# JINXER000/GIE-mapping

Measured on AMD Instinct MI355X. Metric: edt_map_update_throughput, higher is better.
Workload: dtype int32; 1 GPU; 512x512x512 @ 0.05 m, sensor-less hash world (BASELINE config 5): occupied iff hash(x,y,z) < 1 %, full observation, 25 ~; preset=c5, fast_mode=False, tiles=single volume, blocks=360448

## Files before the change

gie-mapping_amd/csrc/gie_api.inc.h:

```cpp
#include <stdio.h>
#include <stdlib.h>
#include <string.h>
#include <math.h>
#include <string>
#include <vector>

enum { GIE_K_CLASSIFY = 0, GIE_K_RAY_REGISTER, GIE_K_RAY_FREE, GIE_K_RAY_FINAL, GIE_K_ALLOC, GIE_K_FUSE, GIE_K_EDT_Y, GIE_K_EDT_X,
       GIE_K_EDT_Z, GIE_K_MARK, GIE_K_FRONTIER, GIE_K_WAVE_A, GIE_K_WAVE_B, GIE_K_WAVE_C, GIE_K_COMMIT, GIE_K_EDT_ZFACES, GIE_K_MARKC, GIE_K_NUM };
#include <cstdio>
#include <unistd.h>
static const char *const gie_kernel_names[GIE_K_NUM] = { "ogm_classify", "ray_register", "ray_free", "ray_finalize", "block_alloc", "fuse",
       "edt_pass_y", "edt_pass_x", "edt_pass_z", "mark", "frontiers", "wave_a", "wave_b", "waves", "commit", "edt_prep", "mark_commit" };

#define GIE_REHASH_PERIOD 64
static thread_local std::string g_gie_err;
static void gie_set_err(const std::string &s) { g_gie_err = s; }
extern "C" const char *gie_last_error(void) { return g_gie_err.c_str(); }

enum gie_owed {
    GIE_OWED_NONE,
    GIE_OWED_FRESH,
    GIE_OWED_STALE
};
struct gie_pivots { int pvt[3], upvt[3], tb0[3]; };
// ... 762 lines not shown
}

extern "C" int gie_step(gie_mapper *m)
{
    int rc = gie_fuse(m); if (rc) return rc;
    rc = gie_batch_edt(m); if (rc) return rc;
    return gie_merge(m);
}

static int gie_fetch_counters(gie_mapper *m)
{
    be_d2h(&m->be, m->h_cnt, m->c.cnt, sizeof(m->h_cnt));
    const int e = m->h_cnt[GIE_CNT_ERR];
    {
        static const int dbg = GIE_SWITCH("GIE_DEBUG_COUNTS", 0);
        if (dbg) fprintf(stderr, "gie counts: tiles known %d, frontier tiles %d, fuse tiles %d, seeds A/B/C %d %d %d, tiles without a read of the stored records %d, tiles caught up %d, lazy tiles written out %d\n", m->h_cnt[GIE_CNT_TL_KNOWN],
                         m->h_cnt[GIE_CNT_TL_FRONT], m->h_cnt[GIE_CNT_TL_FUSE], m->h_cnt[GIE_CNT_SEED_A], m->h_cnt[GIE_CNT_SEED_B], m->h_cnt[GIE_CNT_SEED_C], m->h_cnt[GIE_CNT_TSKIP],
                         m->h_cnt[GIE_CNT_STATE1], m->h_cnt[GIE_CNT_STATE2]);
    }
    if (e & ~GIE_ERRF_BARRIER) {
        std::string s = "device capacity exceeded:";
        if (e & GIE_ERRF_POOL) s += " block pool (raise gie_config.max_blocks)";
        if (e & GIE_ERRF_QUEUE) s += " frontier queue";
        if (e & GIE_ERRF_HASH) s += " hash table";
        gie_set_err(s);
        return GIE_ERR_CAPACITY;
    }
    if (e & GIE_ERRF_BARRIER) {
        be_memset(&m->be, &m->c.cnt[GIE_CNT_ERR], 0, sizeof(int32_t));
        be_sync(&m->be);
        gie_set_err("grid barrier of the wavefront kernel timed out (its workgroups were not all resident: another process is holding the "
                    "device); this map update is incomplete, the next one runs normally");
        return GIE_ERR_TIMEOUT;
// ... 488 lines not shown
```

gie-mapping_amd/csrc/gie_hip.hip:

```cpp
#include <cstdio>
#include <unistd.h>
#include <cstring>
#include <cstdlib>
#include <string>
#include <algorithm>
#include <vector>
#include <hip/hip_runtime.h>
#include <hip/hip_ext.h>
#include <rocprim/rocprim.hpp>
#include "gie_kernels.hip.h"

#define GIE_NEV 8

struct be_state {
    int device;
    int num_cu;
    int cu_total;
    hipStream_t stream;
    hipEvent_t ev[GIE_NEV];
    int ev_set[GIE_NEV];
    void *scan_tmp; size_t scan_bytes;
    void *arena;
    hipEvent_t copy_ev[2];
    hipStream_t side;
// ... 282 lines not shown
{
    constexpr int LP = 64 * CP;
    const size_t tile = ((size_t)c.Z * (TX + 1) + 3) & ~(size_t)3;
    const size_t lds = tile * 4 + (size_t)WAVES * LP * 8 + (size_t)LP * 2 + 16;
    static bool attr_done = false;
    if (!attr_done) {
        GIE_HIP_OK(hipFuncSetAttribute(reinterpret_cast<const void *>(&k_edt_z<CP, TX, WAVES>), hipFuncAttributeMaxDynamicSharedMemorySize, 160 * 1024));
        attr_done = true;
    }
    const int ntx = (c.X + TX - 1) / TX, ntiles = ntx * c.Y;
    int wgs = (int)((160 * 1024) / (lds + 256));
    if (wgs < 1) wgs = 1; if (wgs > 4) wgs = 4;
    int grid = wgs * b->cu_total; if (grid > (ntiles + 1) / 2) grid = (ntiles + 1) / 2;
    GIE_LAUNCH(b, (k_edt_z<CP, TX, WAVES>), dim3(grid), dim3(64 * WAVES), lds, c, ntx, ntiles, full);
}
template <int CP> static void gie_launch_edt_xz(be_state *b, const gie_ctx &c, bool zpass, int full)
{
    if (!zpass) {
        GIE_LAUNCH(b, k_edt_x<CP>, dim3((c.Y + GIE_EDTX_WAVES - 1) / GIE_EDTX_WAVES, c.Z), dim3(64 * GIE_EDTX_WAVES), 0, c);
    } else {
        gie_launch_edt_z<CP, 16, 8>(b, c, full);
    }
}
static void gie_launch_edt_dim(be_state *b, const gie_ctx &c, int L, bool zpass, int full)
{
    if (L <= 64) gie_launch_edt_xz<1>(b, c, zpass, full);
    else if (L <= 128) gie_launch_edt_xz<2>(b, c, zpass, full);
    else if (L <= 256) gie_launch_edt_xz<4>(b, c, zpass, full);
    else if (L <= 512) gie_launch_edt_xz<8>(b, c, zpass, full);
    else gie_launch_edt_xz<16>(b, c, zpass, full);
}
static int be_edt_z_stream(be_state *b, const gie_ctx &c, int full);
static void be_edt_z(be_state *b, const gie_ctx &c, int full) { (void)be_edt_z_stream(b, c, full); gie_launch_edt_dim(b, c, c.Z, true, full); }
template <bool STAGED, class F> static void be_vox_list(be_state *b, const gie_ctx &c, const F &f, const int32_t *list, int count_idx, int always_list, int lx = 64)
{
    static const int mult = GIE_SWITCH("GIE_VOXA_MULT", 32);
    const dim3 g(b->cu_total * mult), t(256);
    if (lx == 32) GIE_LAUNCH(b, (k_voxa<F, STAGED, 32>), g, t, 0, c, f, list, count_idx, always_list);
    else if (lx == 16) GIE_LAUNCH(b, (k_voxa<F, STAGED, 16>), g, t, 0, c, f, list, count_idx, always_list);
    else if (lx == 8) GIE_LAUNCH(b, (k_voxa<F, STAGED, 8>), g, t, 0, c, f, list, count_idx, always_list);
    else GIE_LAUNCH(b, (k_voxa<F, STAGED, 64>), g, t, 0, c, f, list, count_idx, always_list);
}
static void be_markc(be_state *b, const gie_ctx &c, const int32_t *list)
{
    static const int generic = GIE_SWITCH("GIE_MARKC_GENERIC", 0);
    static const int lx = GIE_SWITCH("GIE_MARKC_LX", 32);
    static const int mult = GIE_SWITCH("GIE_VOXA_MULT", 64);
    if (generic) { be_vox_list<true>(b, c, op_markc(), list, GIE_CNT_TL_KNOWN, 0, lx == 16 || lx == 8 || lx == 32 ? lx : 64); return; }
// ... 47 lines not shown
    GIE_LAUNCH(b, k_frontier_faces, dim3(nsum + nface), dim3(64 * GIE_FF_WAVES), 0, c, fp, known, known_idx, nsum);
    static int mult = GIE_SWITCH("GIE_FRONT_MULT", 0);
    if (mult <= 0) {
        int per_cu = 0;
        if (hipOccupancyMaxActiveBlocksPerMultiprocessor(&per_cu, reinterpret_cast<const void *>(&k_frontier_tiles), 64 * GIE_FR_WAVES, 0) != hipSuccess || per_cu < 1) per_cu = 2;
        mult = per_cu;
    }
    GIE_LAUNCH(b, k_frontier_tiles, dim3(b->cu_total * mult), dim3(64 * GIE_FR_WAVES), 0, c, list, count_idx);
}
static void be_edt_z_direct(be_state *b, const gie_ctx &c)
{
    GIE_LAUNCH(b, k_edt_z_direct, dim3(b->cu_total * 16), dim3(256), 0, c);
}
static int be_edt_z_stream(be_state *b, const gie_ctx &c, int full)
{
    if (c.Z < 64 || c.Z > 1024) return 0;
    static const int on = GIE_SWITCH("GIE_ZSTREAM", 1);
    if (!on) return 0;
    const int nxr = (c.X + 63) / 64;
    static const int target = GIE_SWITCH("GIE_ZSTREAM_WAVES", 8);
    const long long want = (long long)b->cu_total * 4 * target;
    int nseg = (int)((want + (long long)nxr * c.Y - 1) / ((long long)nxr * c.Y));
    const int maxseg = c.Z / 64 > 0 ? c.Z / 64 : 1;
    if (nseg > maxseg) nseg = maxseg; if (nseg < 1) nseg = 1;
    int seg_len = ((c.Z + nseg - 1) / nseg + 31) & ~31;
    nseg = (c.Z + seg_len - 1) / seg_len;
    const long long waves = (long long)nxr * nseg * c.Y;
    long long grid = (waves + 3) / 4;
    const long long cap = (long long)b->cu_total * 8 * 4;
    if (grid > cap) grid = cap;
    if (!full && grid < (long long)b->cu_total * 16) grid = (long long)b->cu_total * 16;
    GIE_LAUNCH(b, k_edt_z_stream, dim3((unsigned)grid), dim3(256), 0, c, full, nseg, seg_len);
    return 1;
}
static void be_tile_oldskip(be_state *b, const gie_ctx &c, const int pupvt[3])
{
    const int ntile = c.tfd[0] * c.tfd[1] * c.tfd[2];
    int32_t *const count = &c.cnt[GIE_CNT_STATE1];
    GIE_LAUNCH(b, k_tile_oldskip, dim3((ntile + 255) / 256), dim3(256), 0, c, ntile, c.wc_list[0], count);
    if (c.catchup_fast) GIE_LAUNCH(b, k_coc_catchup_new, dim3(b->cu_total * 8), dim3(256), 0, c, pupvt[0], pupvt[1], pupvt[2], c.wc_list[0], count);
}
static void be_pair_materialise(be_state *b, const gie_ctx &c, int stay)
{
    const int ntile = c.tfd[0] * c.tfd[1] * c.tfd[2];
    int32_t *const count = &c.cnt[GIE_CNT_STATE2];
    GIE_LAUNCH(b, k_pair_lazy_list, dim3((ntile + 255) / 256), dim3(256), 0, c, ntile, stay, c.wc_list[1], count);
    GIE_LAUNCH(b, k_pair_lazy_run, dim3(b->cu_total * 8), dim3(256), 0, c, c.wc_list[1], count);
// ... 17 lines not shown
    be_prof(b, 6, 0);
    static const int y4 = GIE_SWITCH("GIE_EDTY4", 1);
    if (y4 && (c.X & 3) == 0) {
        const int yb = c.Y > 512 ? 32 : 16, nq = (c.Y + yb - 1) / yb;
        const int lanes = (y4 == 3) ? 32 : 16;
        dim3 g4((c.X / 4 + lanes - 1) / lanes, c.Z), b4(lanes, nq);
        if (yb == 16 && lanes == 16) GIE_LAUNCH(b, (k_edt_y4<16, 16>), g4, b4, 0, c);
        else if (yb == 16) GIE_LAUNCH(b, (k_edt_y4<16, 32>), g4, b4, 0, c);
        else if (lanes == 16) GIE_LAUNCH(b, (k_edt_y4<32, 16>), g4, b4, 0, c);
        else GIE_LAUNCH(b, (k_edt_y4<32, 32>), g4, b4, 0, c);
    }
    else if (c.Y <= 256) GIE_LAUNCH(b, (k_edt_y<8, 8>), gy, dim3(GIE_EDTY_COLS, 8), 0, c);
    else if (c.Y <= 512) GIE_LAUNCH(b, (k_edt_y<16, 16>), gy, dim3(GIE_EDTY_COLS, 16), 0, c);
    else GIE_LAUNCH(b, (k_edt_y<32, 16>), gy, dim3(GIE_EDTY_COLS, 16), 0, c);
    be_prof(b, 6, 1);
    be_prof(b, 7, 0); gie_launch_edt_dim(b, c, c.X, false, 1); be_prof(b, 7, 1);
    be_prof(b, 8, 0);
    if (!be_edt_z_stream(b, c, full) && !full) be_edt_z_direct(b, c);
    gie_launch_edt_dim(b, c, c.Z, true, full);
    be_prof(b, 8, 1);

}
static void be_waves(be_state *b, const gie_ctx &c, int with_ab, int record_seeds, int clear_first)
{
    std::lock_guard<std::mutex> lock(g_waves_mutex);
    const int dv = b->device & 63;
    (void)hipSetDevice(b->device);
    const bool chain = g_live_mappers[dv] > 1;
    if (chain) {
        if (g_waves_event_set[dv]) GIE_HIP_OK(hipStreamWaitEvent(b->stream, g_waves_event[dv], 0));
        else { GIE_HIP_OK(hipEventCreateWithFlags(&g_waves_event[dv], hipEventDisableTiming)); g_waves_event_set[dv] = true; }
    }
    if (clear_first) {
        GIE_HIP_OK(hipMemsetAsync(&c.cnt[GIE_CNT_BAR_B], 0, 2 * sizeof(int32_t), b->stream));
// ... 9 lines not shown
```

gie-mapping_amd/csrc/gie_kernels.hip.h:

```cpp
#ifndef GIE_KERNELS_HIP_H
#define GIE_KERNELS_HIP_H

#include <hip/hip_runtime.h>
#include "gie_functors.h"

#if defined(GIE_WAVE_TIMING) || defined(GIE_RAY_TIMING)
#include "../../tools/measure/gie_timing.h"
#endif
#if !defined(GIE_WAVE_TIMING)
#define GIE_TS2(tag, n) do { } while (0)
#define GIE_WPROF_DECL do { } while (0)
#define GIE_WPROF_MARK(base) do { } while (0)
#define GIE_WPROF_ADD(i, v) do { } while (0)
#define GIE_WPROF_END(base) do { } while (0)
#define GIE_WPROF_DRAIN() do { } while (0)
#define GIE_WPROF_SUB(i) do { } while (0)
#define GIE_WPROF_SUBSTART() do { } while (0)
#define GIE_WPROF_DUMP() do { } while (0)
#define GIE_WPROF_CLK() 0ull
#define GIE_WAVE_TIMING_RESET(cond) do { } while (0)
#endif
#if !defined(GIE_RAY_TIMING)
#define GIE_RTS(k) do { } while (0)
#endif
// ... 689 lines not shown

__device__ __forceinline__ int gie_row_compact_push(uint2 *ce, int base, const bool valid, const uint32_t a, const int i, const uint32_t hi16, const int lane, int2 *mb = nullptr)
{
    const unsigned long long m = __ballot(valid);
    if (valid) {
        const int j = base + __popcll(m & ((1ull << lane) - 1ull));
        ce[j] = make_uint2((a << 10) | (uint32_t)j, ((uint32_t)i << 5) | (hi16 << 16));
        if (mb && j < GIE_BAND_MAXK) mb[j] = make_int2(-(i << 11), (int)((((uint32_t)(i * i) + a) << 10) | (uint32_t)j));
    }
    return base + __popcll(m);
}

#ifndef GIE_EDTX_WAVES
#define GIE_EDTX_WAVES 4
#endif
template <int CP>
__global__ __launch_bounds__(64 * GIE_EDTX_WAVES) void k_edt_x(const gie_ctx c)
{
    constexpr int LP = 64 * CP;
    __shared__ __attribute__((aligned(16))) uint2 s_ce[GIE_EDTX_WAVES][LP];
    constexpr bool OVL = LP >= 2 * (GIE_BAND_MAXK + GIE_BAND_PAD) && LP / 2 >= GIE_BAND_MAXK;
    __shared__ __attribute__((aligned(16))) int2 s_mb[OVL ? 1 : GIE_EDTX_WAVES][OVL ? 1 : GIE_BAND_MAXK + GIE_BAND_PAD];
    const int wave = threadIdx.x >> 6, lane = threadIdx.x & 63;
    const int z = blockIdx.y, y = blockIdx.x * GIE_EDTX_WAVES + wave;
    if (!c.zocc[z]) return;
    if (y >= c.Y) return;
    const int X = c.X;
    const size_t row = (size_t)z * c.Y + y;
    const uint16_t *in = c.cy1 + row * X;
    uint2 *ce = s_ce[wave];
    int2 *mb = OVL ? reinterpret_cast<int2 *>(ce + LP / 2) : s_mb[OVL ? 0 : wave];
    int K = 0;
    uint16_t cyv[CP];
#pragma unroll
    for (int m = 0; m < CP; m++) { const int i = 64 * m + lane; cyv[m] = __builtin_nontemporal_load(&in[min(i, X - 1)]); }
    uint32_t *out = c.cxy2 + row * X;
    if (CP >= 4) {
        int kall = 0;
#pragma unroll
// ... 52 lines not shown
        int sj[CP];
        gie_row_argmin<CP>(ce, K, X, lane, sj);
#pragma unroll
        for (int m = 0; m < CP; m++) {
            const uint32_t e = ce[sj[m]].y;
            o[m] = ((e & 0xffffu) >> 5) | (e & 0xffff0000u);
        }
    }
    if (CP >= 4 && (X & 3) == 0) {
#pragma unroll
        for (int m = 0; m < CP; m += 4)
            if (u0 + m < X) *reinterpret_cast<uint4 *>(out + u0 + m) = make_uint4(o[m], o[m + 1 < CP ? m + 1 : m], o[m + 2 < CP ? m + 2 : m], o[m + 3 < CP ? m + 3 : m]);
    } else {
#pragma unroll
        for (int m = 0; m < CP; m++) if (u0 + m < X) out[u0 + m] = o[m];
    }
}

template <int CP, int TX, int WAVES>
__global__ __launch_bounds__(64 * WAVES, (CP <= 8 ? 4 : 2)) void k_edt_z(const gie_ctx c, const int ntiles_x, const int ntiles, const int full)
{
    static_assert(TX == 16 && WAVES == 8, "a workgroup tile spans two 8-voxel tile columns, one column per wave and half");
    if (full == 0 && gie_z_use_lists(c, c.cnt[GIE_CNT_TL_KNOWN])) return;
    const int repair = c.cnt[GIE_CNT_ZSTREAM];
    if (repair && c.cnt[GIE_CNT_ZFAIL] == 0) return;
    constexpr int LP = 64 * CP;
    constexpr int TS = TX + 1;
    constexpr int NT = 64 * WAVES;
    constexpr int ZSTEP = NT / TX;
    constexpr int NLD = (LP + ZSTEP - 1) / ZSTEP;
// ... 189 lines not shown
#define GIE_ZS_C 16
#endif
#define GIE_ZS_W (GIE_ZS_C + 2 * GIE_ZS_R)
#define GIE_ZS_LDAUX 2
#define GIE_ZS_STAUX 2
#define GIE_ZS_NONE 0xb0000000u
#define GIE_ZS_LIMIT ((uint32_t)((GIE_ZS_R + 1) * (GIE_ZS_R + 1)) << 24)
__device__ __forceinline__ uint32_t gie_zs_key(const uint32_t v, const bool plane_ok, const int x8, const int y8, const int j)
{
    const uint32_t ux = (uint32_t)(x8 - (int)(v & 0xffffu)), uy = (uint32_t)(y8 - (int)(v >> 16));
    const int dx = (int)ux - 8, dy = (int)uy - 8;
    const uint32_t a = (uint32_t)(__mul24(dx, dx) + __mul24(dy, dy));
    const bool ok = plane_ok && max(ux, uy) <= 16u && a < (uint32_t)((GIE_ZS_R + 1) * (GIE_ZS_R + 1));
    return ok ? ((a << 24) | ((uint32_t)j << 18) | (ux << 13) | (uy << 8)) : (GIE_ZS_NONE | ((uint32_t)j << 18));
}
__device__ __forceinline__ void gie_edt_z_direct_body(const gie_ctx &c);
#define GIE_ZS_R2 24
__device__ __noinline__ bool gie_zs_wide_trip(const uint32_t *cxy2, uint32_t *bcoc, const unsigned nbytes, const unsigned voff, const unsigned pstride,
                                              const int zc, const int z1, const int Z, const int x, const int y, const bool inx, const uint8_t *occ)
{
    const __amdgpu_buffer_rsrc_t rs_in = __builtin_amdgcn_make_buffer_rsrc(const_cast<uint32_t *>(cxy2), 0, nbytes, 0x00020000);
    const __amdgpu_buffer_rsrc_t rs_out = __builtin_amdgcn_make_buffer_rsrc(bcoc, 0, nbytes, 0x00020000);
    uint32_t best[GIE_ZS_C];
#pragma unroll
    for (int t = 0; t < GIE_ZS_C; t++) best[t] = 0xffffffffu;
    const int lo = max(zc - GIE_ZS_R2, 0), hi = min(zc + GIE_ZS_C + GIE_ZS_R2, Z);
#pragma unroll 1
    for (int i0 = lo; i0 < hi; i0 += 8) {
        uint32_t v[8];
#pragma unroll
// ... 8 lines not shown
            for (int t = 0; t < GIE_ZS_C; t++) { const int d = zc + t - i; best[t] = min(best[t], (min(a + (uint32_t)(d * d), 0x3fffffu) << 10) | (uint32_t)i); }
        }
    }
    uint32_t worst = 0;
#pragma unroll
    for (int t = 0; t < GIE_ZS_C; t++) if (zc + t < z1) worst = max(worst, best[t]);
    if (__any(inx && worst >= ((uint32_t)((GIE_ZS_R2 + 1) * (GIE_ZS_R2 + 1)) << 10))) return false;
#pragma unroll
    for (int t = 0; t < GIE_ZS_C; t++) {
        const int sp = (int)(best[t] & 1023u);
        const uint32_t v = __builtin_amdgcn_raw_buffer_load_b32(rs_in, voff, (unsigned)sp * pstride, 0);
        __builtin_amdgcn_raw_buffer_store_b32(gie_pack_bcoc((int)(v & 0xffffu), (int)(v >> 16), sp), rs_out, (zc + t < z1) ? voff : GIE_BUF_OOB, (unsigned)min(zc + t, Z - 1) * pstride, 0);
    }
    return true;
}
__global__ __launch_bounds__(256, 6) void k_edt_z_stream(const gie_ctx c, const int full, const int nseg, const int seg_len)
{
    __shared__ uint8_t s_occ[1024 + 2 * (32 + 2 * GIE_ZS_R)];
    const int Z = c.Z, X = c.X, Y = c.Y;
    if (full == 0 && gie_z_use_lists(c, c.cnt[GIE_CNT_TL_KNOWN])) { gie_edt_z_direct_body(c); return; }
    if (*c.zcount <= GIE_BAND_MAXK) return;
    if (blockIdx.x == 0 && threadIdx.x == 0) c.cnt[GIE_CNT_ZSTREAM] = 1;
    for (int i = threadIdx.x; i < Z + 2 * GIE_ZS_W; i += 256) { const int z = i - GIE_ZS_W; s_occ[i] = (z >= 0 && z < Z) ? c.zocc[z] : (uint8_t)0; }
    __syncthreads();
    const int lane = threadIdx.x & 63;
    const int nxr = (X + 63) >> 6;
    const int total = nxr * nseg * Y;
    const size_t plane = (size_t)X * Y;
    const unsigned nbytes = (unsigned)((size_t)X * Y * Z * 4u);
    const __amdgpu_buffer_rsrc_t rs_in = __builtin_amdgcn_make_buffer_rsrc(const_cast<uint32_t *>(c.cxy2), 0, nbytes, 0x00020000);
    const __amdgpu_buffer_rsrc_t rs_out = __builtin_amdgcn_make_buffer_rsrc(c.bcoc, 0, nbytes, 0x00020000);
    const unsigned pstride = (unsigned)(plane * 4u);
    for (int w = (int)blockIdx.x * 4 + (int)(threadIdx.x >> 6); w < total; w += (int)gridDim.x * 4) {
        const int xr = w % nxr, seg = (w / nxr) % nseg, y = w / (nxr * nseg);
        const int x = xr * 64 + lane;
        const int z0 = seg * seg_len, z1 = min(Z, z0 + seg_len);
        if (z0 >= Z) continue;
        const unsigned voff = x < X ? (unsigned)(y * X + x) * 4u : GIE_BUF_OOB;
        const int x8 = x + 8, y8 = y + 8;
        uint32_t wk[GIE_ZS_W];
        {
            const int zz = z0 - GIE_ZS_R + lane;
            const unsigned long long pm = __ballot(lane < 2 * GIE_ZS_R && s_occ[zz + GIE_ZS_W] != 0);
            uint32_t v[2 * GIE_ZS_R];
#pragma unroll
            for (int j = 0; j < 2 * GIE_ZS_R; j++) { const int zp = min(max(z0 - GIE_ZS_R + j, 0), Z - 1); v[j] = __builtin_amdgcn_raw_buffer_load_b32(rs_in, voff, (unsigned)zp * pstride, 0); }
#pragma unroll
            for (int j = 0; j < 2 * GIE_ZS_R; j++) wk[j] = gie_zs_key(v[j], (pm >> j) & 1ull, x8, y8, j);
        }
        bool failed = false;
        int wide = 0, wz0 = 0, wz1 = 0;
#pragma unroll 1
        for (int zc = z0; zc < z1; zc += GIE_ZS_C) {
            {
                const int zz = zc + GIE_ZS_R + lane;
                const unsigned long long pm = __ballot(lane < GIE_ZS_C && s_occ[zz + GIE_ZS_W] != 0);
                uint32_t v[GIE_ZS_C];
#pragma unroll
                for (int j = 0; j < GIE_ZS_C; j++) { const int zp = min(zc + GIE_ZS_R + j, Z - 1); v[j] = __builtin_amdgcn_raw_buffer_load_b32(rs_in, voff, (unsigned)zp * pstride, GIE_ZS_LDAUX); }
#pragma unroll
                for (int j = 0; j < GIE_ZS_C; j++) wk[2 * GIE_ZS_R + j] = gie_zs_key(v[j], (pm >> j) & 1ull, x8, y8, 2 * GIE_ZS_R + j);
            }
            uint32_t wlo = 0, whi = 0;
#pragma unroll
            for (int t = 0; t < GIE_ZS_C; t++) {
                const int p = GIE_ZS_R + t;
                uint32_t b = wk[p];
#pragma unroll
                for (int d = 1; d <= GIE_ZS_R; d++) b = min(b, min(wk[p - d], wk[p + d]) + ((uint32_t)(d * d) << 24));
// ... 12 lines not shown
                m0 = max(m0, (uint32_t)__shfl_xor((int)m0, 4)); m1 = max(m1, (uint32_t)__shfl_xor((int)m1, 4));
                if ((lane & 7) == 0 && x < X) {
                    const int t0 = gie_tile_index(c, x, y, zc);
                    __hip_atomic_fetch_max(&c.tbmax[t0], (int32_t)m0, __ATOMIC_RELAXED, __HIP_MEMORY_SCOPE_AGENT);
                    if (zc + 8 < z1) __hip_atomic_fetch_max(&c.tbmax[t0 + c.tfd[0] * c.tfd[1]], (int32_t)m1, __ATOMIC_RELAXED, __HIP_MEMORY_SCOPE_AGENT);
                }
            }
            if (__any(x < X && worst >= GIE_ZS_LIMIT)) {
                if (wide == 2) { failed = true; break; }
                if (wide == 0) wz0 = zc; else wz1 = zc;
                wide++;
            }
#pragma unroll
            for (int j = 0; j < 2 * GIE_ZS_R; j++) wk[j] = wk[GIE_ZS_C + j] - ((uint32_t)GIE_ZS_C << 18);
        }
        if (!failed && wide > 0) failed = !gie_zs_wide_trip(c.cxy2, c.bcoc, nbytes, voff, pstride, wz0, z1, Z, x, y, x < X, s_occ + GIE_ZS_W);
        if (!failed && wide > 1) failed = !gie_zs_wide_trip(c.cxy2, c.bcoc, nbytes, voff, pstride, wz1, z1, Z, x, y, x < X, s_occ + GIE_ZS_W);
        if (failed && lane < 4) {
            const int tx16 = xr * 4 + lane;
            if (tx16 * 16 < X) c.zredo[(size_t)y * ((X + 15) >> 4) + tx16] = 1u;
            if (lane == 0) atomicAdd(&c.cnt[GIE_CNT_ZFAIL], 1);
        }
    }
}

#define GIE_PREP_WAVES 16
__global__ __launch_bounds__(64 * GIE_PREP_WAVES) void k_edt_prep(const gie_ctx c, const int ncol)
{
    if (blockIdx.x == 0 && threadIdx.x < 64) {
        uint8_t f[16];
#pragma unroll
        for (int i = 0; i < 16; i++) { const int z = 64 * i + (int)threadIdx.x; f[i] = c.zocc[min(z, c.Z - 1)]; }
        int k = 0;
#pragma unroll
        for (int i = 0; i < 16; i++) {
            const int z = 64 * i + (int)threadIdx.x;
// ... 1914 lines not shown
```

gie-mapping_amd/csrc/gie_ops.h:

```cpp
#ifndef GIE_OPS_H
#define GIE_OPS_H

#include "gie_types.h"

#ifndef GIE_PLATFORM_DEFINED
#include "gie_platform.h"
#endif

GIE_DEV void gie_push64(const gie_ctx &c, uint64_t *q, int32_t *counter, int cap, uint64_t v)
{
    const int i = gie_aadd32(counter, 1);
    if (i < cap) gie_st(&q[i], v); else gie_aor32(&c.cnt[GIE_CNT_ERR], GIE_ERRF_QUEUE);
}
GIE_DEV void gie_push64a(const gie_ctx &c, uint64_t *q, gie_vaddr *qaddr, int32_t *counter, int cap, uint64_t v, gie_vaddr a)
{
    const int i = gie_aadd32(counter, 1);
    if (i < cap) { gie_st(&q[i], v); gie_st(&qaddr[i], a); } else gie_aor32(&c.cnt[GIE_CNT_ERR], GIE_ERRF_QUEUE);
}
GIE_DEV void gie_push64a_wave(const gie_ctx &c, uint64_t *q, gie_vaddr *qaddr, int32_t *counter, int cap, bool push, uint64_t v, gie_vaddr a)
{
    const unsigned long long m = __ballot(push);
    if (!m) return;
    const int lane = __lane_id(), leader = __ffsll((long long)m) - 1;
    int base = 0;
// ... 700 lines not shown
}
GIE_DEV int gie_frontier_voxel(const gie_ctx &c, int x, int y, int z)
{
    const int id = gie_lid(c, x, y, z);
    if (c.glb_type[id] == GIE_VOX_UNKNOWN) return 0;
    gie_frontier_st s;
    gie_frontier_load1(c, id, x, y, z, s);
    return gie_frontier_finish(c, id, x, y, z, s);
}

GIE_DEV int gie_batch_dist_direct(const gie_ctx &c, int x, int y, int z)
{
    const int K = *c.zcount;
    const size_t plane = (size_t)c.X * c.Y, o = (size_t)y * c.X + x;
    int best = c.max_width * c.max_width;
    for (int j = 0; j < K; j += 8) {
        int zj[8]; uint32_t v[8];
#pragma unroll
        for (int u = 0; u < 8; u++) zj[u] = c.zlist[j + u < K ? j + u : K - 1];
#pragma unroll
        for (int u = 0; u < 8; u++) v[u] = c.cxy2[(size_t)zj[u] * plane + o];
#pragma unroll
        for (int u = 0; u < 8; u++) {
            const int dx = x - (int)(v[u] & 0xffffu), dy = y - (int)(v[u] >> 16), dz = z - zj[u];
            const int d = dx * dx + dy * dy + dz * dz;
            best = d < best ? d : best;
        }
    }
    return best;
}
// ... 526 lines not shown
```

gie-mapping_amd/csrc/gie_types.h:

```cpp
#ifndef GIE_TYPES_H
#define GIE_TYPES_H

#include <stdint.h>
#include "../../include/gie.h"
#include "../../include/gie_math.h"

#define GIE_VB 8
#define GIE_VBSZ 512
typedef long long gie_vaddr;

#define GIE_PAIR_DIST_SHIFT 42
#define GIE_PAIR_NEW (1ull << 41)
#define GIE_PAIR_PAR_MASK ((1ull << 41) - 1ull)
#define GIE_PAR_NONE GIE_PAIR_PAR_MASK
#define GIE_NOPROP 0xffffffffffffffffull

GIE_HD uint64_t gie_pair_make(int dist, uint64_t par) { return ((uint64_t)(uint32_t)dist << GIE_PAIR_DIST_SHIFT) | (par & GIE_PAIR_PAR_MASK); }
GIE_HD int gie_pair_dist(uint64_t p) { return (int)(p >> GIE_PAIR_DIST_SHIFT); }
GIE_HD uint64_t gie_pair_par(uint64_t p) { return p & GIE_PAIR_PAR_MASK; }
GIE_HD uint64_t gie_pack_wr(int x, int y, int z) { return (uint64_t)(uint32_t)x | ((uint64_t)(uint32_t)y << 14) | ((uint64_t)(uint32_t)z << 28); }
GIE_HD void gie_unpack_wr(uint64_t id, int *x, int *y, int *z)
{
    *x = (int)(id & 0x3fff); *y = (int)((id >> 14) & 0x3fff); *z = (int)((id >> 28) & 0x1fff);
    if ((id & GIE_PAIR_PAR_MASK) == GIE_PAR_NONE) *z = 0x3fff;
// ... 119 lines not shown
    uint64_t *qa, *qb;
    gie_vaddr *qa_a, *qb_a;
    int32_t *qc[2];
    int qcap_ab, qcap_c;
    int32_t *cnt;
    int32_t *lvl_next, *lvl_vis;
    int32_t *wc_list[2];
    int32_t *wc_flag[2];
    const int32_t *gate;
} gie_ctx;
#define GIE_GATE_CLOSED(c) ((c).gate != nullptr && *(const volatile int32_t *)(c).gate == 0)

enum {
    GIE_CNT_A = 0, GIE_CNT_B, GIE_CNT_C,
    GIE_CNT_TL_SWEPT,
    GIE_CNT_FREE4, GIE_CNT_FREE5,
    GIE_CNT_LV0, GIE_CNT_LV1, GIE_CNT_LV2,
    GIE_CNT_ERR,
    GIE_CNT_NEWBLK,
    GIE_CNT_VIS_A, GIE_CNT_VIS_B, GIE_CNT_VIS_C,
    GIE_CNT_LVL_A, GIE_CNT_LVL_B, GIE_CNT_LVL_C,
    GIE_CNT_FRONT_B, GIE_CNT_FRONT_C,
    GIE_CNT_SEED_A, GIE_CNT_SEED_B, GIE_CNT_SEED_C,
    GIE_CNT_ZSTREAM,
    GIE_CNT_ZFAIL,
    GIE_CNT_STATE1, GIE_CNT_STATE2,
    GIE_CNT_FRAME_END = 28,
    GIE_CNT_TOT_A = 28, GIE_CNT_TOT_B = 30, GIE_CNT_TOT_C = 32,
    GIE_CNT_BAR_B = 34,
    GIE_CNT_BAR_C = 35,
    GIE_CNT_NEWLIST = 36,
// ... 107 lines not shown
```

Baseline: 90190 Mvoxels/s.

## Fuse X-pass into Z-stream EDT using cy1 LDS rows, redo failed slabs

When the streamed Z pass will run, the X pass kernel now exits early. The Z-stream kernel instead builds its keys directly from the 16-bit cy1 plane through LDS row windows, and the wide trips read cy1 the same way. This is meant to drop the separate X-pass write and read of cxy2. Rows whose slabs fail are recomputed by a new redo X kernel, and tile max bounds are raised. gie_batch_dist_direct can now read the streamed bcoc result instead of scanning all z-slices. This adds complexity and possible correctness risk around the fallback paths.

```diff
diff --git a/gie-mapping_amd/csrc/gie_api.inc.h b/gie-mapping_amd/csrc/gie_api.inc.h
--- a/gie-mapping_amd/csrc/gie_api.inc.h
+++ b/gie-mapping_amd/csrc/gie_api.inc.h
@@ -800,9 +800,9 @@
     const int e = m->h_cnt[GIE_CNT_ERR];
     {
         static const int dbg = GIE_SWITCH("GIE_DEBUG_COUNTS", 0);
-        if (dbg) fprintf(stderr, "gie counts: tiles known %d, frontier tiles %d, fuse tiles %d, seeds A/B/C %d %d %d, tiles without a read of the stored records %d, tiles caught up %d, lazy tiles written out %d\n", m->h_cnt[GIE_CNT_TL_KNOWN],
+        if (dbg) fprintf(stderr, "gie counts: tiles known %d, frontier tiles %d, fuse tiles %d, seeds A/B/C %d %d %d, tiles without a read of the stored records %d, tiles caught up %d, lazy tiles written out %d, pass Z streamed %d (wide trips %d, slabs given up %d)\n", m->h_cnt[GIE_CNT_TL_KNOWN],
                          m->h_cnt[GIE_CNT_TL_FRONT], m->h_cnt[GIE_CNT_TL_FUSE], m->h_cnt[GIE_CNT_SEED_A], m->h_cnt[GIE_CNT_SEED_B], m->h_cnt[GIE_CNT_SEED_C], m->h_cnt[GIE_CNT_TSKIP],
-                         m->h_cnt[GIE_CNT_STATE1], m->h_cnt[GIE_CNT_STATE2]);
+                         m->h_cnt[GIE_CNT_STATE1], m->h_cnt[GIE_CNT_STATE2], m->h_cnt[GIE_CNT_ZSTREAM], m->h_cnt[GIE_CNT_ZWIDE], m->h_cnt[GIE_CNT_ZFAIL]);
     }
     if (e & ~GIE_ERRF_BARRIER) {
         std::string s = "device capacity exceeded:";
diff --git a/gie-mapping_amd/csrc/gie_hip.hip b/gie-mapping_amd/csrc/gie_hip.hip
--- a/gie-mapping_amd/csrc/gie_hip.hip
+++ b/gie-mapping_amd/csrc/gie_hip.hip
@@ -320,24 +320,38 @@
     int grid = wgs * b->cu_total; if (grid > (ntiles + 1) / 2) grid = (ntiles + 1) / 2;
     GIE_LAUNCH(b, (k_edt_z<CP, TX, WAVES>), dim3(grid), dim3(64 * WAVES), lds, c, ntx, ntiles, full);
 }
-template <int CP> static void gie_launch_edt_xz(be_state *b, const gie_ctx &c, bool zpass, int full)
-{
-    if (!zpass) {
-        GIE_LAUNCH(b, k_edt_x<CP>, dim3((c.Y + GIE_EDTX_WAVES - 1) / GIE_EDTX_WAVES, c.Z), dim3(64 * GIE_EDTX_WAVES), 0, c);
+template <int CP> static void gie_launch_edt_xz(be_state *b, const gie_ctx &c, bool zpass, int full, int zs_fused = 0, bool redo = false)
+{
+    if (redo) {
+        GIE_LAUNCH(b, k_edt_x_redo<CP>, dim3(b->cu_total * 8), dim3(64 * GIE_EDTX_WAVES), 0, c);
+    } else if (!zpass) {
+        GIE_LAUNCH(b, k_edt_x<CP>, dim3((c.Y + GIE_EDTX_WAVES - 1) / GIE_EDTX_WAVES, c.Z), dim3(64 * GIE_EDTX_WAVES), 0, c, zs_fused, full);
     } else {
         gie_launch_edt_z<CP, 16, 8>(b, c, full);
     }
 }
-static void gie_launch_edt_dim(be_state *b, const gie_ctx &c, int L, bool zpass, int full)
-{
-    if (L <= 64) gie_launch_edt_xz<1>(b, c, zpass, full);
-    else if (L <= 128) gie_launch_edt_xz<2>(b, c, zpass, full);
-    else if (L <= 256) gie_launch_edt_xz<4>(b, c, zpass, full);
-    else if (L <= 512) gie_launch_edt_xz<8>(b, c, zpass, full);
-    else gie_launch_edt_xz<16>(b, c, zpass, full);
+static void gie_launch_edt_dim(be_state *b, const gie_ctx &c, int L, bool zpass, int full, int zs_fused = 0, bool redo = false)
+{
+    if (L <= 64) gie_launch_edt_xz<1>(b, c, zpass, full, zs_fused, redo);
+    else if (L <= 128) gie_launch_edt_xz<2>(b, c, zpass, full, zs_fused, redo);
+    else if (L <= 256) gie_launch_edt_xz<4>(b, c, zpass, full, zs_fused, redo);
+    else if (L <= 512) gie_launch_edt_xz<8>(b, c, zpass, full, zs_fused, redo);
+    else gie_launch_edt_xz<16>(b, c, zpass, full, zs_fused, redo);
+}
+static int be_zs_mode(const gie_ctx &c)
+{
+    if (c.Z < 64 || c.Z > 1024) return 0;
+    static const int on = GIE_SWITCH("GIE_ZSTREAM", 1);
+    static const int fused = GIE_SWITCH("GIE_ZS_FUSED", 1);
+    return on ? ((fused && (c.X & 1) == 0) ? 2 : 1) : 0;
 }
 static int be_edt_z_stream(be_state *b, const gie_ctx &c, int full);
-static void be_edt_z(be_state *b, const gie_ctx &c, int full) { (void)be_edt_z_stream(b, c, full); gie_launch_edt_dim(b, c, c.Z, true, full); }
+static void be_edt_z_rest(be_state *b, const gie_ctx &c, int full, int zs)
+{
+    if (zs == 2) gie_launch_edt_dim(b, c, c.X, false, full, 0, true);
+    gie_launch_edt_dim(b, c, c.Z, true, full);
+}
+static void be_edt_z(be_state *b, const gie_ctx &c, int full) { be_edt_z_rest(b, c, full, be_edt_z_stream(b, c, full) ? be_zs_mode(c) : 0); }
 template <bool STAGED, class F> static void be_vox_list(be_state *b, const gie_ctx &c, const F &f, const int32_t *list, int count_idx, int always_list, int lx = 64)
 {
     static const int mult = GIE_SWITCH("GIE_VOXA_MULT", 32);
@@ -415,9 +429,8 @@
 }
 static int be_edt_z_stream(be_state *b, const gie_ctx &c, int full)
 {
-    if (c.Z < 64 || c.Z > 1024) return 0;
-    static const int on = GIE_SWITCH("GIE_ZSTREAM", 1);
-    if (!on) return 0;
+    const int zs = be_zs_mode(c);
+    if (!zs) return 0;
     const int nxr = (c.X + 63) / 64;
     static const int target = GIE_SWITCH("GIE_ZSTREAM_WAVES", 8);
     const long long want = (long long)b->cu_total * 4 * target;
@@ -431,7 +444,8 @@
     const long long cap = (long long)b->cu_total * 8 * 4;
     if (grid > cap) grid = cap;
     if (!full && grid < (long long)b->cu_total * 16) grid = (long long)b->cu_total * 16;
-    GIE_LAUNCH(b, k_edt_z_stream, dim3((unsigned)grid), dim3(256), 0, c, full, nseg, seg_len);
+    if (zs == 2) GIE_LAUNCH(b, k_edt_z_stream<true>, dim3((unsigned)grid), dim3(256), 0, c, full, nseg, seg_len, zs);
+    else GIE_LAUNCH(b, k_edt_z_stream<false>, dim3((unsigned)grid), dim3(256), 0, c, full, nseg, seg_len, zs);
     return 1;
 }
 static void be_tile_oldskip(be_state *b, const gie_ctx &c, const int pupvt[3])
@@ -479,10 +493,12 @@
     else if (c.Y <= 512) GIE_LAUNCH(b, (k_edt_y<16, 16>), gy, dim3(GIE_EDTY_COLS, 16), 0, c);
     else GIE_LAUNCH(b, (k_edt_y<32, 16>), gy, dim3(GIE_EDTY_COLS, 16), 0, c);
     be_prof(b, 6, 1);
-    be_prof(b, 7, 0); gie_launch_edt_dim(b, c, c.X, false, 1); be_prof(b, 7, 1);
+    const int zs = be_zs_mode(c);
+    be_prof(b, 7, 0); gie_launch_edt_dim(b, c, c.X, false, full, zs == 2 ? zs : 0); be_prof(b, 7, 1);
     be_prof(b, 8, 0);
-    if (!be_edt_z_stream(b, c, full) && !full) be_edt_z_direct(b, c);
-    gie_launch_edt_dim(b, c, c.Z, true, full);
+    const int zl = be_edt_z_stream(b, c, full);
+    if (!zl && !full) be_edt_z_direct(b, c);
+    be_edt_z_rest(b, c, full, zl ? zs : 0);
     be_prof(b, 8, 1);
 
 }
diff --git a/gie-mapping_amd/csrc/gie_kernels.hip.h b/gie-mapping_amd/csrc/gie_kernels.hip.h
--- a/gie-mapping_amd/csrc/gie_kernels.hip.h
+++ b/gie-mapping_amd/csrc/gie_kernels.hip.h
@@ -727,15 +727,18 @@
 #ifndef GIE_EDTX_WAVES
 #define GIE_EDTX_WAVES 4
 #endif
+GIE_HD int gie_zs_takes(const gie_ctx &c, const int zs, const int full)
+{
+    return zs && !(full == 0 && gie_z_use_lists(c, c.cnt[GIE_CNT_TL_KNOWN])) && *c.zcount > GIE_BAND_MAXK;
+}
 template <int CP>
-__global__ __launch_bounds__(64 * GIE_EDTX_WAVES) void k_edt_x(const gie_ctx c)
+__device__ __forceinline__ void gie_edt_x_row(const gie_ctx &c, const int y, const int z)
 {
     constexpr int LP = 64 * CP;
     __shared__ __attribute__((aligned(16))) uint2 s_ce[GIE_EDTX_WAVES][LP];
     constexpr bool OVL = LP >= 2 * (GIE_BAND_MAXK + GIE_BAND_PAD) && LP / 2 >= GIE_BAND_MAXK;
     __shared__ __attribute__((aligned(16))) int2 s_mb[OVL ? 1 : GIE_EDTX_WAVES][OVL ? 1 : GIE_BAND_MAXK + GIE_BAND_PAD];
     const int wave = threadIdx.x >> 6, lane = threadIdx.x & 63;
-    const int z = blockIdx.y, y = blockIdx.x * GIE_EDTX_WAVES + wave;
     if (!c.zocc[z]) return;
     if (y >= c.Y) return;
     const int X = c.X;
@@ -818,6 +821,33 @@
     } else {
 #pragma unroll
         for (int m = 0; m < CP; m++) if (u0 + m < X) out[u0 + m] = o[m];
+    }
+}
+template <int CP>
+__global__ __launch_bounds__(64 * GIE_EDTX_WAVES) void k_edt_x(const gie_ctx c, const int zs, const int full)
+{
+    if (zs && gie_zs_takes(c, zs, full)) return;
+    gie_edt_x_row<CP>(c, blockIdx.x * GIE_EDTX_WAVES + (int)(threadIdx.x >> 6), blockIdx.y);
+}
+template <int CP>
+__global__ __launch_bounds__(64 * GIE_EDTX_WAVES) void k_edt_x_redo(const gie_ctx c)
+{
+    if (c.cnt[GIE_CNT_ZFAIL] == 0) return;
+    const int K = *c.zcount, Y = c.Y, lane = threadIdx.x & 63;
+    const int nw = (int)gridDim.x * GIE_EDTX_WAVES, w0 = (int)blockIdx.x * GIE_EDTX_WAVES + (int)(threadIdx.x >> 6);
+    const int ntx = (c.X + 15) >> 4, nkc = (K + 7) >> 3;
+#pragma unroll 1
+    for (int u = w0; u < Y * nkc; u += nw) {
+        const int uu = __builtin_amdgcn_readfirstlane(u);
+        const int y = uu / nkc, k0 = (uu % nkc) * 8;
+        bool f = false;
+        for (int i = lane; i < ntx; i += 64) f |= c.zredo[(size_t)y * ntx + i] != 0u;
+        if (!__any(f)) continue;
+#pragma unroll 1
+        for (int k = k0; k < min(k0 + 8, K); k++) {
+            gie_wave_sync();
+            gie_edt_x_row<CP>(c, y, c.zlist[k]);
+        }
     }
 }
 
@@ -1037,6 +1067,59 @@
     const bool ok = plane_ok && max(ux, uy) <= 16u && a < (uint32_t)((GIE_ZS_R + 1) * (GIE_ZS_R + 1));
     return ok ? ((a << 24) | ((uint32_t)j << 18) | (ux << 13) | (uy << 8)) : (GIE_ZS_NONE | ((uint32_t)j << 18));
 }
+#define GIE_ZS_XW (64 + 2 * GIE_ZS_R)
+#define GIE_ZS_ROWS 8
+#ifndef GIE_ZS_CHAINS
+#define GIE_ZS_CHAINS 4
+#endif
+#ifndef GIE_ZS_FUSED_WGS
+#define GIE_ZS_FUSED_WGS 7
+#endif
+__device__ __forceinline__ uint32_t gie_zs_col(const uint32_t cy, const bool ok, const int y8)
+{
+    const uint32_t uy = (uint32_t)(y8 - (int)cy);
+    const int dy = (int)uy - 8;
+    return (ok && uy <= 16u) ? (((uint32_t)__mul24(dy, dy) << 24) | (uy << 8)) : GIE_ZS_NONE;
+}
+typedef __attribute__((address_space(3))) uint32_t gie_lds_u32;
+__device__ __forceinline__ uint32_t gie_zs_fused_key(const gie_lds_u32 *row, const int j)
+{
+    uint32_t m = 0xffffffffu;
+#pragma unroll
+    for (int k = 0; k <= 2 * GIE_ZS_R; k++) m = min(m, row[k] + (((uint32_t)((k - GIE_ZS_R) * (k - GIE_ZS_R)) << 24) | ((uint32_t)(15 + k) << 13)));
+    return m < GIE_ZS_LIMIT ? ((m ^ (31u << 13)) | ((uint32_t)j << 18)) : (GIE_ZS_NONE | ((uint32_t)j << 18));
+}
+template <int NP, int JB, int AUX>
+__device__ __forceinline__ void gie_zs_fused_keys(uint32_t (&wk)[GIE_ZS_W], uint32_t (*srow)[GIE_ZS_XW], const __amdgpu_buffer_rsrc_t rs, const unsigned vo,
+                                                  const unsigned ps2, const int zfirst, const int Z, const unsigned long long pm, const bool ok0, const bool ok1, const int y8, const int lane)
+{
+    static_assert(NP % GIE_ZS_ROWS == 0, "whole batches of rows");
+    uint32_t v[NP];
+#pragma unroll
+    for (int j = 0; j < NP; j++) {
+        const unsigned so = (unsigned)min(max(__builtin_amdgcn_readfirstlane(zfirst) + j, 0), Z - 1) * ps2;
+        v[j] = __builtin_amdgcn_raw_buffer_load_b32(rs, vo, so, AUX);
+    }
+#pragma unroll
+    for (int j0 = 0; j0 < NP; j0 += GIE_ZS_ROWS) {
+#pragma unroll
+        for (int j = j0; j < j0 + GIE_ZS_ROWS; j++) {
+            const bool po = (pm >> j) & 1ull;
+            if (lane < GIE_ZS_XW / 2)
+                *reinterpret_cast<uint2 *>(&srow[j - j0][2 * lane]) = make_uint2(gie_zs_col(v[j] & 0xffffu, po && ok0, y8), gie_zs_col(v[j] >> 16, po && ok1, y8));
+        }
+        gie_wave_sync();
+        gie_lds_u32 *rp[GIE_ZS_CHAINS];
+#pragma unroll
+        for (int q = 0; q < GIE_ZS_CHAINS; q++) rp[q] = (gie_lds_u32 *)&srow[0][lane];
+#pragma unroll
+        for (int j = j0; j < j0 + GIE_ZS_ROWS; j++) {
+            wk[JB + j] = gie_zs_fused_key(rp[j % GIE_ZS_CHAINS] + (j - j0) * GIE_ZS_XW, JB + j);
+            asm volatile("" : "+v"(rp[j % GIE_ZS_CHAINS]) : "v"(wk[JB + j]));
+        }
+        gie_wave_sync();
+    }
+}
 __device__ __forceinline__ void gie_edt_z_direct_body(const gie_ctx &c);
 #define GIE_ZS_R2 24
 __device__ __noinline__ bool gie_zs_wide_trip(const uint32_t *cxy2, uint32_t *bcoc, const unsigned nbytes, const unsigned voff, const unsigned pstride,
@@ -1075,12 +1158,71 @@
     }
     return true;
 }
-__global__ __launch_bounds__(256, 6) void k_edt_z_stream(const gie_ctx c, const int full, const int nseg, const int seg_len)
+#define GIE_ZS_XW2 (64 + 2 * GIE_ZS_R2)
+static_assert(2 * GIE_ZS_XW2 <= GIE_ZS_ROWS * GIE_ZS_XW, "the wide trip's row and its cy fit the wave's LDS rows");
+__device__ __forceinline__ bool gie_zs_wide_trip_fused(const __amdgpu_buffer_rsrc_t rs_cy, const __amdgpu_buffer_rsrc_t rs_out, gie_lds_u32 *srow, const unsigned voff,
+                                                       const unsigned pstride, const unsigned ps2, const int zc, const int z1, const int Z, const int x0, const int x,
+                                                       const int y, const int X, const uint8_t *occ, const int lane)
+{
+    const int xa = x0 - GIE_ZS_R2 + lane, xb = x0 + 64 - GIE_ZS_R2 + lane;
+    const bool oka = xa >= 0 && xa < X, okb = lane < 2 * GIE_ZS_R2 && xb < X;
+    const unsigned voa = oka ? (unsigned)(y * X + xa) * 2u : GIE_BUF_OOB, vob = okb ? (unsigned)(y * X + xb) * 2u : GIE_BUF_OOB;
+    gie_lds_u32 *sq = srow, *scy = srow + GIE_ZS_XW2;
+    uint32_t best[GIE_ZS_C], bc[GIE_ZS_C];
+#pragma unroll
+    for (int t = 0; t < GIE_ZS_C; t++) { best[t] = 0xffffffffu; bc[t] = GIE_BCOC_NONE; }
+    const int lo = max(zc - GIE_ZS_R2, 0), hi = min(zc + GIE_ZS_C + GIE_ZS_R2, Z);
+#pragma unroll 1
+    for (int i0 = lo; i0 < hi; i0 += 8) {
+        uint16_t va[8], vb[8];
+#pragma unroll
+        for (int k = 0; k < 8; k++) {
+            const unsigned so = (unsigned)min(i0 + k, Z - 1) * ps2;
+            va[k] = __builtin_amdgcn_raw_buffer_load_b16(rs_cy, voa, so, 0);
+            vb[k] = __builtin_amdgcn_raw_buffer_load_b16(rs_cy, vob, so, 0);
+        }
+#pragma unroll
+        for (int k = 0; k < 8; k++) {
+            const int i = i0 + k;
+            if (i >= hi || !occ[i]) continue;
+            {
+                const int da = y - (int)va[k], db = y - (int)vb[k];
+                sq[lane] = (oka && va[k] != 0xffffu) ? ((uint32_t)(da * da) << 6) : 0x3fffffc0u; scy[lane] = va[k];
+                if (lane < 2 * GIE_ZS_R2) { sq[64 + lane] = (okb && vb[k] != 0xffffu) ? ((uint32_t)(db * db) << 6) : 0x3fffffc0u; scy[64 + lane] = vb[k]; }
+            }
+            gie_wave_sync();
+            uint32_t m = 0xffffffffu;
+#pragma unroll
+            for (int q = 0; q <= 2 * GIE_ZS_R2; q++) m = min(m, sq[lane + q] + (((uint32_t)((q - GIE_ZS_R2) * (q - GIE_ZS_R2)) << 6) | (uint32_t)q));
+            const int q = (int)(m & 63u);
+            const uint32_t cc = gie_pack_bcoc(x - GIE_ZS_R2 + q, (int)scy[lane + q], i);
+            gie_wave_sync();
+            const uint32_t a = min(m >> 6, 0x3fffffu);
+#pragma unroll
+            for (int t = 0; t < GIE_ZS_C; t++) {
+                const int d = zc + t - i;
+                const uint32_t nb = (min(a + (uint32_t)(d * d), 0x3fffffu) << 10) | (uint32_t)i;
+                if (nb < best[t]) { best[t] = nb; bc[t] = cc; }
+            }
+        }
+    }
+    uint32_t worst = 0;
+#pragma unroll
+    for (int t = 0; t < GIE_ZS_C; t++) if (zc + t < z1) worst = max(worst, best[t]);
+    if (__any(x < X && worst >= ((uint32_t)((GIE_ZS_R2 + 1) * (GIE_ZS_R2 + 1)) << 10))) return false;
+#pragma unroll
+    for (int t = 0; t < GIE_ZS_C; t++)
+        __builtin_amdgcn_raw_buffer_store_b32(bc[t], rs_out, (zc + t < z1) ? voff : GIE_BUF_OOB, (unsigned)min(zc + t, Z - 1) * pstride, 0);
+    return true;
+}
+template <bool FUSED>
+__global__ __launch_bounds__(256, FUSED ? GIE_ZS_FUSED_WGS : 6) void k_edt_z_stream(const gie_ctx c, const int full, const int nseg, const int seg_len, const int zs)
 {
     __shared__ uint8_t s_occ[1024 + 2 * (32 + 2 * GIE_ZS_R)];
     const int Z = c.Z, X = c.X, Y = c.Y;
     if (full == 0 && gie_z_use_lists(c, c.cnt[GIE_CNT_TL_KNOWN])) { gie_edt_z_direct_body(c); return; }
-    if (*c.zcount <= GIE_BAND_MAXK) return;
+    if (!gie_zs_takes(c, zs, full)) return;
+    __shared__ __attribute__((aligned(16))) uint32_t s_row[FUSED ? 4 : 1][FUSED ? GIE_ZS_ROWS : 1][GIE_ZS_XW];
     if (blockIdx.x == 0 && threadIdx.x == 0) c.cnt[GIE_CNT_ZSTREAM] = 1;
     for (int i = threadIdx.x; i < Z + 2 * GIE_ZS_W; i += 256) { const int z = i - GIE_ZS_W; s_occ[i] = (z >= 0 && z < Z) ? c.zocc[z] : (uint8_t)0; }
     __syncthreads();
@@ -1090,17 +1232,27 @@
     const size_t plane = (size_t)X * Y;
     const unsigned nbytes = (unsigned)((size_t)X * Y * Z * 4u);
     const __amdgpu_buffer_rsrc_t rs_in = __builtin_amdgcn_make_buffer_rsrc(const_cast<uint32_t *>(c.cxy2), 0, nbytes, 0x00020000);
+    const __amdgpu_buffer_rsrc_t rs_cy = __builtin_amdgcn_make_buffer_rsrc(const_cast<uint16_t *>(c.cy1), 0, nbytes / 2u, 0x00020000);
     const __amdgpu_buffer_rsrc_t rs_out = __builtin_amdgcn_make_buffer_rsrc(c.bcoc, 0, nbytes, 0x00020000);
-    const unsigned pstride = (unsigned)(plane * 4u);
+    const unsigned pstride = (unsigned)(plane * 4u), pstride2 = (unsigned)(plane * 2u);
     for (int w = (int)blockIdx.x * 4 + (int)(threadIdx.x >> 6); w < total; w += (int)gridDim.x * 4) {
-        const int xr = w % nxr, seg = (w / nxr) % nseg, y = w / (nxr * nseg);
+        const int wu = __builtin_amdgcn_readfirstlane(w);
+        const int xr = wu % nxr, seg = (wu / nxr) % nseg, y = wu / (nxr * nseg);
         const int x = xr * 64 + lane;
         const int z0 = seg * seg_len, z1 = min(Z, z0 + seg_len);
         if (z0 >= Z) continue;
         const unsigned voff = x < X ? (unsigned)(y * X + x) * 4u : GIE_BUF_OOB;
         const int x8 = x + 8, y8 = y + 8;
         uint32_t wk[GIE_ZS_W];
-        {
+        const int xa = xr * 64 - GIE_ZS_R + 2 * lane;
+        const bool oka = lane < GIE_ZS_XW / 2 && xa >= 0 && xa < X, okb = lane < GIE_ZS_XW / 2 && xa + 1 >= 0 && xa + 1 < X;
+        const unsigned vpa = (oka || okb) ? (unsigned)(y * X + xa) * 2u : GIE_BUF_OOB;
+        uint32_t (*srow)[GIE_ZS_XW] = s_row[FUSED ? (threadIdx.x >> 6) : 0];
+        if (FUSED) {
+            const int zz = z0 - GIE_ZS_R + lane;
+            const unsigned long long pm = __ballot(lane < 2 * GIE_ZS_R && s_occ[zz + GIE_ZS_W] != 0);
+            gie_zs_fused_keys<2 * GIE_ZS_R, 0, 0>(wk, srow, rs_cy, vpa, pstride2, z0 - GIE_ZS_R, Z, pm, oka, okb, y8, lane);
+        } else {
             const int zz = z0 - GIE_ZS_R + lane;
             const unsigned long long pm = __ballot(lane < 2 * GIE_ZS_R && s_occ[zz + GIE_ZS_W] != 0);
             uint32_t v[2 * GIE_ZS_R];
@@ -1113,7 +1265,11 @@
         int wide = 0, wz0 = 0, wz1 = 0;
 #pragma unroll 1
         for (int zc = z0; zc < z1; zc += GIE_ZS_C) {
-            {
+            if (FUSED) {
+                const int zz = zc + GIE_ZS_R + lane;
+                const unsigned long long pm = __ballot(lane < GIE_ZS_C && s_occ[zz + GIE_ZS_W] != 0);
+                gie_zs_fused_keys<GIE_ZS_C, 2 * GIE_ZS_R, GIE_ZS_LDAUX>(wk, srow, rs_cy, vpa, pstride2, zc + GIE_ZS_R, Z, pm, oka, okb, y8, lane);
+            } else {
                 const int zz = zc + GIE_ZS_R + lane;
                 const unsigned long long pm = __ballot(lane < GIE_ZS_C && s_occ[zz + GIE_ZS_W] != 0);
                 uint32_t v[GIE_ZS_C];
@@ -1156,12 +1312,24 @@
 #pragma unroll
             for (int j = 0; j < 2 * GIE_ZS_R; j++) wk[j] = wk[GIE_ZS_C + j] - ((uint32_t)GIE_ZS_C << 18);
         }
-        if (!failed && wide > 0) failed = !gie_zs_wide_trip(c.cxy2, c.bcoc, nbytes, voff, pstride, wz0, z1, Z, x, y, x < X, s_occ + GIE_ZS_W);
-        if (!failed && wide > 1) failed = !gie_zs_wide_trip(c.cxy2, c.bcoc, nbytes, voff, pstride, wz1, z1, Z, x, y, x < X, s_occ + GIE_ZS_W);
-        if (failed && lane < 4) {
-            const int tx16 = xr * 4 + lane;
-            if (tx16 * 16 < X) c.zredo[(size_t)y * ((X + 15) >> 4) + tx16] = 1u;
-            if (lane == 0) atomicAdd(&c.cnt[GIE_CNT_ZFAIL], 1);
+        if (wide > 0 && lane == 0) atomicAdd(&c.cnt[GIE_CNT_ZWIDE], wide);
+        if (FUSED) {
+#pragma unroll 1
+            for (int k = 0; k < wide && !failed; k++)
+                failed = !gie_zs_wide_trip_fused(rs_cy, rs_out, (gie_lds_u32 *)&srow[0][0], voff, pstride, pstride2, __builtin_amdgcn_readfirstlane(k ? wz1 : wz0), z1, Z, xr * 64, x, y, X,
+                                                 s_occ + GIE_ZS_W, lane);
+        } else {
+            if (!failed && wide > 0) failed = !gie_zs_wide_trip(c.cxy2, c.bcoc, nbytes, voff, pstride, wz0, z1, Z, x, y, x < X, s_occ + GIE_ZS_W);
+            if (!failed && wide > 1) failed = !gie_zs_wide_trip(c.cxy2, c.bcoc, nbytes, voff, pstride, wz1, z1, Z, x, y, x < X, s_occ + GIE_ZS_W);
+        }
+        if (failed) {
+            if (lane < 4) {
+                const int tx16 = xr * 4 + lane;
+                if (tx16 * 16 < X) c.zredo[(size_t)y * ((X + 15) >> 4) + tx16] = 1u;
+                if (lane == 0) atomicAdd(&c.cnt[GIE_CNT_ZFAIL], 1);
+            }
+            if ((lane & 7) == 0 && x < X)
+                for (int zt = z0; zt < z1; zt += 8) __hip_atomic_fetch_max(&c.tbmax[gie_tile_index(c, x, y, zt)], (int32_t)((GIE_ZS_R + 1) * (GIE_ZS_R + 1)), __ATOMIC_RELAXED, __HIP_MEMORY_SCOPE_AGENT);
         }
     }
 }
diff --git a/gie-mapping_amd/csrc/gie_ops.h b/gie-mapping_amd/csrc/gie_ops.h
--- a/gie-mapping_amd/csrc/gie_ops.h
+++ b/gie-mapping_amd/csrc/gie_ops.h
@@ -738,6 +738,11 @@
     const int K = *c.zcount;
     const size_t plane = (size_t)c.X * c.Y, o = (size_t)y * c.X + x;
     int best = c.max_width * c.max_width;
+    if (c.cnt[GIE_CNT_ZSTREAM] && c.zredo[(size_t)y * ((c.X + 15) >> 4) + (x >> 4)] == 0u) {
+        const uint32_t bc = c.bcoc[(size_t)z * plane + o];
+        const int d = gie_d2(x, y, z, (int)(bc & 1023u), (int)((bc >> 10) & 1023u), (int)(bc >> 20));
+        return d < best ? d : best;
+    }
     for (int j = 0; j < K; j += 8) {
         int zj[8]; uint32_t v[8];
 #pragma unroll
diff --git a/gie-mapping_amd/csrc/gie_types.h b/gie-mapping_amd/csrc/gie_types.h
--- a/gie-mapping_amd/csrc/gie_types.h
+++ b/gie-mapping_amd/csrc/gie_types.h
@@ -157,7 +157,8 @@
 enum {
     GIE_CNT_A = 0, GIE_CNT_B, GIE_CNT_C,
     GIE_CNT_TL_SWEPT,
-    GIE_CNT_FREE4, GIE_CNT_FREE5,
+    GIE_CNT_ZWIDE,
+    GIE_CNT_FREE5,
     GIE_CNT_LV0, GIE_CNT_LV1, GIE_CNT_LV2,
     GIE_CNT_ERR,
     GIE_CNT_NEWBLK,
```

New measurement: 98530 Mvoxels/s (median of 6 runs). +9.2%, better.
